# Nikhil-AI-Labs/Image-Super-Resolution

Measured on AMD Instinct MI355X. Metric: SR output megapixels/s (x4, 510x340 LR -> 2040x1360, full 4-expert + 7-phase fusion), higher is better.
Workload: dtype f32 (GEMM/conv products as 3-term split-bf16 MFMA, fp32 accumulate)

## Files before the change

image-super-resolution_amd/csrc/ffsr_attn.hip:

```cpp
#include "ffsr_common.h"

namespace {

struct WinArgs {
  const float* qkv;
  const float* bias;
  float* out;
  int ldq, ldo, C, H, W, ws, shift, heads, hd, hdp, masked;
  float scale;
};

__device__ __forceinline__ int region_id(int p, int n, int ws, int shift) {
  return p < n - ws ? 0 : (p < n - shift ? 1 : 2);
}

template <int DT, int QT>
__global__ __launch_bounds__(256, (QT == 1 ? (DT == 1 ? 4 : (DT == 2 ? 3 : 2)) : (DT <= 2 ? 2 : 1))) void window_attn_kernel(WinArgs p) {
  extern __shared__ __attribute__((aligned(16))) float lds[];
  constexpr int NGMAX = 4 * DT;
  constexpr int WS = 16, N = WS * WS;
  const int QS = p.hdp + 4;
  float* KV = lds;
  int* tok_pix = reinterpret_cast<int*>(KV + 128 * QS + 64);
  int* tok_reg = tok_pix + N;
// ... 525 lines not shown
  for (int d = 0; d < HD; ++d) {
    q[d] = row[d];
    k[d] = row[heads * HD + d];
    Vs[lane][d] = row[2 * heads * HD + d];
  }
  const float kn = inv_norm(k, HD);
#pragma unroll
  for (int d = 0; d < HD; ++d) Ks[lane][d] = k[d] * kn;
  if (lane < NA) {
    const int ay = wy * AW + lane / AW, ax = wx * AW + lane % AW;
    const float* ar = anchor + (((size_t)b * (H / 2) + ay) * (W / 2) + ax) * lda + head * HD;
    float a[HD];
#pragma unroll
    for (int d = 0; d < HD; ++d) a[d] = ar[d];
    const float an = inv_norm(a, HD);
#pragma unroll
    for (int d = 0; d < HD; ++d) As[lane][d] = a[d] * an;
  }
  __syncthreads();
  {
    const int a = lane & 15, kq = lane >> 4;
    const float l1 = logit1[head];
    float s[16];
    float m = -3.0e38f;
#pragma unroll
    for (int jj = 0; jj < 16; ++jj) {
      const int j = kq * 16 + jj;
      float acc = 0.f;
#pragma unroll
      for (int d = 0; d < HD; ++d) acc = fmaf(As[a][d], Ks[j][d], acc);
      acc = acc * l1 + bias1T[((size_t)head * N + j) * NA + a];
      s[jj] = acc;
      m = fmaxf(m, acc);
    }
    m = fmaxf(m, __shfl_xor(m, 16, 64));
    m = fmaxf(m, __shfl_xor(m, 32, 64));
    float sum = 0.f;
#pragma unroll
    for (int jj = 0; jj < 16; ++jj) {
      s[jj] = expf(s[jj] - m);
      sum += s[jj];
    }
    sum += __shfl_xor(sum, 16, 64);
    sum += __shfl_xor(sum, 32, 64);
    const float inv = 1.0f / sum;
#pragma unroll
    for (int jj = 0; jj < 16; ++jj) P1[a][kq * 16 + jj] = s[jj] * inv;
  }
  __syncthreads();
  for (int i = lane; i < NA * HD; i += 64) {
    const int a = i / HD, d = i - a * HD;
    float acc = 0.f;
    for (int j = 0; j < N; ++j) acc = fmaf(P1[a][j], Vs[j][d], acc);
    Gs[a][d] = acc;
  }
  __syncthreads();
  const float qn = inv_norm(q, HD) * logit2[head];
  float s2[NA];
  float m2 = -3.0e38f;
#pragma unroll
  for (int a = 0; a < NA; ++a) {
    float acc = 0.f;
#pragma unroll
    for (int d = 0; d < HD; ++d) acc = fmaf(q[d], As[a][d], acc);
    acc = acc * qn + bias2T[((size_t)head * NA + a) * N + lane];
    s2[a] = acc;
    m2 = fmaxf(m2, acc);
  }
  float sum2 = 0.f;
#pragma unroll
  for (int a = 0; a < NA; ++a) {
    s2[a] = expf(s2[a] - m2);
    sum2 += s2[a];
  }
  const float inv2 = 1.0f / sum2;
  float* orow = out + pix * ldo + ocol0 + head * HD;
#pragma unroll
  for (int d = 0; d < HD; ++d) {
    float acc = 0.f;
#pragma unroll
    for (int a = 0; a < NA; ++a) acc = fmaf(s2[a], Gs[a][d], acc);
    orow[d] = acc * inv2;
  }
}

template <int T>
__global__ __launch_bounds__(256) void pixel_mha_kernel(
    const float* __restrict__ qkv, int ldq, float* __restrict__ out, int ldo, long long S,
                                 int E, int heads, unsigned drop_thr, float keep_scale, unsigned long long seed) {
  constexpr int HD = 16;
  long long idx = (long long)blockIdx.x * blockDim.x + threadIdx.x;
  if (idx >= S * T * heads) return;
  const int h = (int)(idx % heads);
  const long long st = idx / heads;
  const long long seq = st / T;
  const float* qrow = qkv + st * ldq + h * HD;
  float q[HD];
#pragma unroll
  for (int d = 0; d < HD; d += 4) {
    floatx4 v = *reinterpret_cast<const floatx4*>(qrow + d);
    q[d] = v[0] * 0.25f; q[d + 1] = v[1] * 0.25f; q[d + 2] = v[2] * 0.25f; q[d + 3] = v[3] * 0.25f;
  }
  float s[T];
  float m = -3.0e38f;
#pragma unroll
  for (int j = 0; j < T; ++j) {
    const float* krow = qkv + (seq * T + j) * ldq + E + h * HD;
    float acc = 0.f;
#pragma unroll
    for (int d = 0; d < HD; d += 4) {
      floatx4 v = *reinterpret_cast<const floatx4*>(krow + d);
      acc = fmaf(q[d], v[0], acc); acc = fmaf(q[d + 1], v[1], acc);
      acc = fmaf(q[d + 2], v[2], acc); acc = fmaf(q[d + 3], v[3], acc);
    }
    s[j] = acc;
    m = fmaxf(m, acc);
  }
  float sum = 0.f;
#pragma unroll
  for (int j = 0; j < T; ++j) {
    s[j] = expf(s[j] - m);
    sum += s[j];
  }
  const float inv = 1.0f / sum;
  float o[HD];
#pragma unroll
  for (int d = 0; d < HD; ++d) o[d] = 0.f;
#pragma unroll
  for (int j = 0; j < T; ++j) {
    const float* vrow = qkv + (seq * T + j) * ldq + 2 * E + h * HD;
    float pj = s[j] * inv;
    if (drop_thr) {
      const unsigned long long e = (((unsigned long long)seq * heads + h) * T + (unsigned long long)(st - seq * T)) * T + j;
      pj = ffsr_rng_u32(seed, e) >= drop_thr ? pj * keep_scale : 0.f;
    }
#pragma unroll
    for (int d = 0; d < HD; d += 4) {
      floatx4 v = *reinterpret_cast<const floatx4*>(vrow + d);
      o[d] = fmaf(pj, v[0], o[d]); o[d + 1] = fmaf(pj, v[1], o[d + 1]);
      o[d + 2] = fmaf(pj, v[2], o[d + 2]); o[d + 3] = fmaf(pj, v[3], o[d + 3]);
    }
  }
  float* orow = out + st * ldo + h * HD;
#pragma unroll
  for (int d = 0; d < HD; d += 4) {
    floatx4 v = {o[d], o[d + 1], o[d + 2], o[d + 3]};
    *reinterpret_cast<floatx4*>(orow + d) = v;
  }
}

inline bool grid_ok(long long y) { return y > 0 && y <= 65535; }

}

#define ST ((hipStream_t)stream)

extern "C" int ffsr_window_attn_f32(const float* qkv, int ldq, const float* bias, float* out, int ldo, int B, int H, int W,
                                    int C, int heads, int ws, int shift, float scale, int variant, void* stream) {
  FFSR_CHECK(qkv && bias && out && B > 0 && heads > 0 && C % heads == 0);
  FFSR_CHECK(ws > 0 && H % ws == 0 && W % ws == 0 && (ws * ws) % 64 == 0 && ws * ws <= 256);
  FFSR_CHECK(shift >= 0 && shift < ws && ldq >= 3 * C && ldo >= C);
  const int hd = C / heads;
  FFSR_CHECK(hd <= 128);
  WinArgs a;
  a.qkv = qkv; a.bias = bias; a.out = out; a.ldq = ldq; a.ldo = ldo; a.C = C; a.H = H; a.W = W; a.ws = ws;
  a.shift = shift; a.heads = heads; a.hd = hd; a.hdp = (hd + 7) / 8 * 8; a.masked = shift > 0; a.scale = scale;
// ... 2 lines not shown
  FFSR_CHECK(grid_ok((H / ws) * (W / ws) * B));
  if (variant == 0 || variant == 4) {
    const int KS = (hd + 15) / 16, DTx = (KS + 1) / 2;
    const size_t ldsx = (size_t)2 * 64 * (KS * 32 + 16) + (size_t)2 * DTx * 32 * 136 + N * 4 + N +
                        (size_t)(2 * ws - 1) * (2 * ws - 1) * 4;
    const bool wide = variant == 4;
    dim3 gridx((unsigned)(heads * (H / ws) * (W / ws) * B * (wide ? 1 : 2)));
#define LAUNCH_X3(K)                                                                                                  \
  {                                                                                                                   \
    if (ldsx > 64 * 1024) {                                                                                           \
      (void)hipFuncSetAttribute((const void*)window_attn_x3_kernel<K, 4>, hipFuncAttributeMaxDynamicSharedMemorySize, \
                                (int)ldsx);                                                                           \
      (void)hipFuncSetAttribute((const void*)window_attn_x3_kernel<K, 8>, hipFuncAttributeMaxDynamicSharedMemorySize, \
                                (int)ldsx);                                                                           \
    }                                                                                                                 \
    if (wide) FFSR_LAUNCH((window_attn_x3_kernel<K, 8>), gridx, dim3(512), ldsx, ST, a);                        \
    else FFSR_LAUNCH((window_attn_x3_kernel<K, 4>), gridx, dim3(256), ldsx, ST, a);                             \
  }
    switch (KS) {
      case 1: LAUNCH_X3(1); break;
      case 2: LAUNCH_X3(2); break;
      case 3: LAUNCH_X3(3); break;
      case 4: LAUNCH_X3(4); break;
      case 5: LAUNCH_X3(5); break;
      case 6: LAUNCH_X3(6); break;
      case 7: LAUNCH_X3(7); break;
      default: LAUNCH_X3(8); break;
    }
#undef LAUNCH_X3
    return ffsr_launch_status();
  }
  const size_t lds = (size_t)(128 * (a.hdp + 4) + 64) * 4 + 2 * N * 4 + (size_t)(2 * ws - 1) * (2 * ws - 1) * 4;
  FFSR_CHECK(lds <= 160 * 1024);
  const int DT = (hd + 31) / 32;
  const int QT = variant == 2 ? 2 : 1;
  dim3 grid(heads, (H / ws) * (W / ws) * B, QT == 1 ? 2 : 1);
#define LAUNCH_WIN(D, Q)                                                                                            \
  {                                                                                                                 \
    if (lds > 64 * 1024)                                                                                            \
      (void)hipFuncSetAttribute((const void*)window_attn_kernel<D, Q>, hipFuncAttributeMaxDynamicSharedMemorySize, \
                                (int)lds);                                                                          \
    FFSR_LAUNCH((window_attn_kernel<D, Q>), grid, dim3(256), lds, ST, a);                                     \
  }
  switch (DT * 10 + QT) {
    case 11: LAUNCH_WIN(1, 1); break;
    case 12: LAUNCH_WIN(1, 2); break;
    case 21: LAUNCH_WIN(2, 1); break;
    case 22: LAUNCH_WIN(2, 2); break;
    case 31: LAUNCH_WIN(3, 1); break;
    case 32: LAUNCH_WIN(3, 2); break;
    case 41: LAUNCH_WIN(4, 1); break;
    default: LAUNCH_WIN(4, 2); break;
  }
#undef LAUNCH_WIN
  return ffsr_launch_status();
}

extern "C" int ffsr_grl_window_attn_f32(const float* qkv, int ldq, int col0, const float* biasT, const float* logit,
                                        float* out, int ldo, int ocol0, int B, int H, int W, int heads, int hd, int shift,
                                        void* stream) {
  FFSR_CHECK(qkv && biasT && logit && out && B > 0 && H % 8 == 0 && W % 8 == 0 && heads > 0 && shift >= 0 && shift < 8);
  dim3 grid((unsigned)((H / 8) * (W / 8) * B * heads));
  switch (hd) {
    case 30: FFSR_LAUNCH(grl_window_kernel<30>, grid, dim3(64), 0, ST, qkv, ldq, col0, biasT, logit, out, ldo, ocol0, H, W, heads, shift); break;
    case 10: FFSR_LAUNCH(grl_window_kernel<10>, grid, dim3(64), 0, ST, qkv, ldq, col0, biasT, logit, out, ldo, ocol0, H, W, heads, shift); break;
    default: return FFSR_EINVAL;
  }
  return ffsr_launch_status();
}

extern "C" int ffsr_grl_stripe_attn_f32(const float* qkv, int ldq, int col0, const float* anchor, int lda,
                                        const float* bias1T, const float* bias2T, const float* logit1, const float* logit2,
                                        float* out, int ldo, int ocol0, int B, int H, int W, int heads, int hd, void* stream) {
  FFSR_CHECK(qkv && anchor && bias1T && bias2T && logit1 && logit2 && out && B > 0 && H % 8 == 0 && W % 8 == 0 && heads > 0);
  dim3 grid((unsigned)((H / 8) * (W / 8) * B * heads));
  switch (hd) {
    case 30: FFSR_LAUNCH(grl_stripe_kernel<30>, grid, dim3(64), 0, ST, qkv, ldq, col0, anchor, lda, bias1T, bias2T, logit1, logit2, out, ldo, ocol0, H, W, heads); break;
    case 10: FFSR_LAUNCH(grl_stripe_kernel<10>, grid, dim3(64), 0, ST, qkv, ldq, col0, anchor, lda, bias1T, bias2T, logit1, logit2, out, ldo, ocol0, H, W, heads); break;
    default: return FFSR_EINVAL;
  }
  return ffsr_launch_status();
}

extern "C" int ffsr_pixel_mha_f32(const float* qkv, int ldq, float* out, int ldo, long long S, int T, int E, int heads,
                                  float p_drop, long long seed,
                                  void* stream) {
  FFSR_CHECK(qkv && out && S > 0 && heads > 0 && E == heads * 16 && (ldq % 4) == 0 && (ldo % 4) == 0);
  FFSR_CHECK(((uintptr_t)qkv & 15) == 0 && ((uintptr_t)out & 15) == 0);
  FFSR_CHECK(p_drop >= 0.f && p_drop < 1.f);
  const unsigned thr = ffsr_drop_threshold(p_drop);
  const float ks = 1.0f / (1.0f - p_drop);
  long long n = S * T * heads;
  dim3 grid((unsigned)((n + 255) / 256));
  switch (T) {
    case 9: FFSR_LAUNCH(pixel_mha_kernel<9>, grid, dim3(256), 0, ST, qkv, ldq, out, ldo, S, E, heads, thr, ks, (unsigned long long)seed); break;
    case 4: FFSR_LAUNCH(pixel_mha_kernel<4>, grid, dim3(256), 0, ST, qkv, ldq, out, ldo, S, E, heads, thr, ks, (unsigned long long)seed); break;
    default: return FFSR_EINVAL;
  }
  return ffsr_launch_status();
}
```

image-super-resolution_amd/ops.py:

```python
from __future__ import annotations

import math
import os
from dataclasses import dataclass
from typing import Optional

import torch

from . import hip

ACT_NONE, ACT_GELU, ACT_RELU, ACT_LRELU, ACT_SIGMOID, ACT_SILU = range(6)

_ENV_MODE = os.environ.get("FFSR_GEMM_MODE", "bf16x3")
GEMM_MODE = "bf16x3" if _ENV_MODE == "bf16" else _ENV_MODE


WEIGHT_LO = os.environ.get("FFSR_WEIGHT_LO", "1") != "0"


def set_weight_lo(on: bool):
    global WEIGHT_LO
    WEIGHT_LO = bool(on)


# ... 728 lines not shown
    B, H, W, C = x.shape
    n = max(1, min(256, H * W // 64))
    part = torch.empty(B, n, C, device=x.device)
    out = torch.empty(B, C, device=x.device)
    hip.call("ffsr_channel_attention_f32", _ptr(x), ld(x), _ptr(part), n, _ptr(a1.wgt), a1.wgt.shape[1], _ptr(a1.bias),
             _ptr(a3.wgt), a3.wgt.shape[1], _ptr(a3.bias), _ptr(out), B, H * W, C, a1.N, _stream())
    return out


@dataclass
class DwConv:
    w: torch.Tensor
    bias: Optional[torch.Tensor]
    KH: int
    KW: int
    ph: int
    pw: int


def pack_dwconv(w: torch.Tensor, b, device, pad=None) -> DwConv:
    C, one, KH, KW = w.shape
    assert one == 1
    ph, pw = (KH // 2, KW // 2) if pad is None else pad
    return DwConv(w.detach().float().reshape(C, KH * KW).t().contiguous().to(device),
                  None if b is None else b.detach().float().contiguous().to(device), KH, KW, ph, pw)


def dwconv2d(x, dw: DwConv, act=ACT_NONE, out=None):
    B, H, W, C = x.shape
    if out is None:
        out = _like(x)
    hip.call("ffsr_dwconv2d_f32", _ptr(x), ld(x), _ptr(dw.w), _ptr(dw.bias), _ptr(out), ld(out), B, H, W, C, dw.KH,
             dw.KW, dw.ph, dw.pw, act, _stream())
    return out


def dw3x3_gate_pool(x, dw: DwConv):
    B, H, W, C2 = x.shape
    C = C2 // 2
    out = new_map(B, H, W, C, x.device)
    n = _nchunk_gate(H * W)
    part = torch.empty(B, n, C, device=x.device)
    pooled = torch.empty(B, C, device=x.device)
    hip.call("ffsr_dw3x3_gate_pool_f32", _ptr(x), ld(x), _ptr(dw.w), _ptr(dw.bias), _ptr(out), ld(out), _ptr(pooled),
             _ptr(part), B, H, W, C, n, _stream())
    return out, pooled


def bilinear(x, Ho, Wo, mul=1.0, out=None, accumulate=False):
    B, Hi, Wi, C = x.shape
    if out is None:
        out = new_map(B, Ho, Wo, C, x.device)
    hip.call("ffsr_bilinear_f32", _ptr(x), ld(x), _ptr(out), ld(out), B, Hi, Wi, Ho, Wo, C, float(mul),
             int(accumulate), _stream())
    return out


def bicubic_up(x, scale=4, out=None):
    B, H, W, C = x.shape
    if out is None:
        out = new_map(B, H * scale, W * scale, C, x.device)
    hip.call("ffsr_bicubic_up_f32", _ptr(x), ld(x), _ptr(out), ld(out), B, H, W, C, scale, _stream())
    return out


def avgpool2(x, out=None):
    B, H, W, C = x.shape
    if out is None:
        out = new_map(B, H // 2, W // 2, C, x.device)
    hip.call("ffsr_avgpool2_f32", _ptr(x), ld(x), _ptr(out), ld(out), B, H, W, C, _stream())
    return out


def window_attn(qkv, bias, B, H, W, C, heads, ws, shift, scale, out=None, variant=None):
    if out is None:
        out = torch.empty(B * H * W, C, device=qkv.device)
    if variant is None:
        variant = 0 if GEMM_MODE == "bf16x3" else 3
    hip.call("ffsr_window_attn_f32", _ptr(qkv), _mat(qkv)[3], _ptr(bias), _ptr(out), _mat(out)[3], B, H, W, C, heads,
             ws, shift, float(scale), variant, _stream())
    return out


def grl_window_attn(qkv, col0, biasT, logit, out, ocol0, B, H, W, heads, hd, shift):
    hip.call("ffsr_grl_window_attn_f32", _ptr(qkv), _mat(qkv)[3], col0, _ptr(biasT), _ptr(logit), _ptr(out),
             _mat(out)[3], ocol0, B, H, W, heads, hd, shift, _stream())
    return out


def grl_stripe_attn(qkv, col0, anchor, bias1T, bias2T, logit1, logit2, out, ocol0, B, H, W, heads, hd):
    hip.call("ffsr_grl_stripe_attn_f32", _ptr(qkv), _mat(qkv)[3], col0, _ptr(anchor), ld(anchor), _ptr(bias1T),
             _ptr(bias2T), _ptr(logit1), _ptr(logit2), _ptr(out), _mat(out)[3], ocol0, B, H, W, heads, hd, _stream())
    return out


def pixel_mha(qkv, S, T, E, heads, out=None, p_drop=0.0, seed=0):
    if out is None:
        out = torch.empty(S * T, E, device=qkv.device)
    hip.call("ffsr_pixel_mha_f32", _ptr(qkv), _mat(qkv)[3], _ptr(out), _mat(out)[3], S, T, E, heads, float(p_drop), int(seed),
             _stream())
    return out


def scan_chunk(L: int, waves_per_chunk: int = 24) -> int:
    if L >= 64 * 1024:
        best = None
        for c in range(192, 513, 8):
            n = (L + c - 1) // c
            cost = -(-(n * waves_per_chunk) // 4096) * c
            if best is None or cost < best[0]:
                best = (cost, c)
        return best[1]
    c = 32
    while c * 2 <= min(1024, L // 512):
        c *= 2
    return c


SCAN_PAIRS = os.environ.get("FFSR_SCAN_PAIRS", "0") == "1"


def selective_scan4(u, xdbl, dtw, dtb, A, Dv, B, H, W, Dm, R, chunk=None, pairs=None):
    L = H * W
    pairs = (SCAN_PAIRS and L >= 16384) if pairs is None else pairs
    nk = 2 if pairs else 4
    chunk = chunk or scan_chunk(L, nk * B * ((Dm + 63) // 64))
    nchunk = (L + chunk - 1) // chunk
    y = torch.empty(nk, B * L, Dm, device=u.device)
    hstate = torch.empty(B, nk, nchunk, Dm, 16, device=u.device)
    decay = torch.empty_like(hstate)
    hip.call("ffsr_selective_scan4_pairs_f32" if pairs else "ffsr_selective_scan4_f32", _ptr(u), _mat(u)[3], _ptr(xdbl), _mat(xdbl)[3], _ptr(dtw), _ptr(dtb), _ptr(A),
             _ptr(Dv), _ptr(y), Dm, _ptr(hstate), _ptr(decay), B, H, W, Dm, R, 16, chunk, _stream())
    return y


def mamba_norm_gate(y4, z, gamma, beta, eps=1e-5, out=None, out_planes=None, want_f32=True):
    nd, M, C = y4.shape
    assert nd in (2, 4)
    if out_planes is True:
        out_planes = Planes(1, 1, M, C, y4.device)
    if out is None and (want_f32 or out_planes is None):
        out = torch.empty(M, C, device=y4.device)
    hip.call("ffsr_mamba_norm_gate_planes_f32" if nd == 4 else "ffsr_mamba_norm_gate_pairs_f32", _ptr(y4), M * C, C, _ptr(z), _mat(z)[3], _ptr(gamma), _ptr(beta), float(eps),
             _ptr(out), 0 if out is None else _mat(out)[3], None if out_planes is None else _ptr(out_planes.hi),
             None if out_planes is None else _ptr(out_planes.lo), 0 if out_planes is None else out_planes.Cp, M, C, _stream())
    if out_planes is not None:
        return (out, out_planes) if out is not None else out_planes
    return out


def dct_bands(img, D, masks, scale, bands):
    B, H, W, _ = img.shape
    hip.call("ffsr_dct_bands_f32", _ptr(img), ld(img), _ptr(D), _ptr(masks), _ptr(scale), _ptr(bands), 36, B, H, W,
             _stream())


def dwt_db4(img, lo, hi):
    B, H, W, _ = img.shape
    Hd, Wd = (H + 6) // 2 + 1, (W + 6) // 2 + 1
    sub = zeros(B, Hd, Wd, 16, device=img.device)
    hip.call("ffsr_dwt_db4_f32", _ptr(img), ld(img), _ptr(lo), _ptr(hi), _ptr(sub), B, H, W, _stream())
    return sub


def fft_bands(img, twW, twH, mask, scale, bands):
    B, H, W, _ = img.shape
    work = torch.empty(10 * B * 3 * H * (W // 2 + 1), device=img.device)
    hip.call("ffsr_fft_bands_f32", _ptr(img), ld(img), _ptr(twW), _ptr(twH), _ptr(mask), _ptr(scale), _ptr(work),
             _ptr(bands), 36, B, H, W, _stream())


def selector_gates(raw, diff, temperature):
    B, h, w, _ = raw.shape
    gates = torch.empty(B, h, w, 4, device=raw.device)
# ... 92 lines not shown
```

include/ffsr.h:

```cpp
#ifndef FFSR_H
#define FFSR_H

#ifdef __cplusplus
extern "C" {
#endif

#define FFSR_OK 0
#define FFSR_EINVAL (-1)
#define FFSR_ELAUNCH (-2)

int ffsr_conv2d_f32(const float* in, const float* wgt, const float* bias, float* out, const float* res,
                    const float* cvec, const float* rvec, const float* akscale, int B, int H, int W, int Cin, int ldi,
                    int N, int ldo, int ldr, int KH, int KW, int stride, int pad_h, int pad_w, int act, float slope,
                    float cscale, float rscale, int shuffle, int akrows, int tile_hint, void* stream);

int ffsr_set_gemm_terms(int terms);

int ffsr_conv2d_bf16x3(const float* in, const void* wgt_hi, const void* wgt_lo, int ldw, int n_rows_padded,
                       const float* zeros, const float* bias, float* out, const float* res, const float* cvec,
                       const float* rvec, const float* akscale, int B, int H, int W, int Cin, int ldi, int N, int ldo,
                       int ldr, int KH, int KW, int stride, int pad_h, int pad_w, int act, float slope, float cscale,
                       float rscale, int shuffle, int akrows, int bn, void* stream);

int ffsr_conv2d_planes(const void* a_hi, const void* a_lo, int Cp, const void* wgt_hi, const void* wgt_lo,
// ... 7 lines not shown
                       const float* be2, const float* res2, int ldr2, float* out, int ldo, void* out_hi, void* out_lo,
                       int ldp, long long M, int K, int N, int steps, int mode, int pre_ln, float eps1, float eps2,
                       float cscale, float rscale, int waves, void* stream);

int ffsr_tok_chain_tail_f32(const float* x, int ldx, const void* w1, const float* b1, const void* w2, const float* b2,
                            const float* res, int ldr, float* out, int ldo, long long M, int K, int N, int steps, int mode,
                            int pre_ln, float eps1, const void* w3, const float* b3, const float* res3, int ldr3, float* out3,
                            int ldo3, int N3, int act3, float slope3, float cscale3, float rscale3, int waves, void* stream);

int ffsr_tok_head_chain_f32(const float* a, int lda, const float* ascale, const void* w0, const float* b0, const float* g0,
                            const float* be0, float eps0, const float* hres, int ldhr, const float* hres2, int ldhr2,
                            const float* hvec2, int rows_per_batch, const void* w1, const float* b1, const void* w2,
                            const float* b2, const float* g2, const float* be2, float eps2, float* out, int ldo, void* out_hi,
                            void* out_lo, int ldp, long long M, int K, int steps, int mode, int pre_ln, float eps1,
                            const void* w3, const float* b3, const float* res3, int ldr3, float* out3, int ldo3, int N3,
                            int act3, float slope3, float cscale3, float rscale3, int waves, void* stream);

int ffsr_tok_proj_f32(const float* x, long long xstride, int xdirs, int ldx, const float* z, int ldz, const float* pg,
                      const float* pb, float peps, const void* w0, const float* b0, const float* cvec, const float* res,
                      int ldr, const float* rvec, const float* g2, const float* be2, float eps2, float* out, int ldo,
                      int out_pre_ln, void* out_hi, void* out_lo, int ldp, long long M, int K, int N, float cscale,
                      float rscale, int waves, void* stream);

int ffsr_tok_gemm_f32(const float* x, int ldx, const void* w1, const float* b1, const float* cvec, float* out, int ldo,
                      void* out_hi, void* out_lo, int ldp, long long M, int K, int N, int pre_ln, float eps1, int act,
                      float slope, float cscale, int waves, void* stream);

int ffsr_split_planes(const float* x, int ldx, void* hi, void* lo, int ldp, long long M, int C, void* stream);

int ffsr_layernorm_f32(const float* x, int ldx, const float* gamma, const float* beta, float eps, float* out, int ldo,
                       const float* res1, int ldr1, const float* res2, int ldr2, int M, int C, void* stream);

int ffsr_layernorm_planes_f32(const float* x, int ldx, const float* gamma, const float* beta, float eps, float* out,
                              int ldo, void* out_hi, void* out_lo, int ldp, const float* res1, int ldr1,
                              const float* res2, int ldr2, const float* res2_vec, int rows_per_batch, int M, int C,
                              void* stream);

int ffsr_unary_f32(const float* x, int ldx, float* out, int ldo, long long M, int C, int act, float slope, float pre,
                   float alpha, float beta, const float* cscale, const float* cbias, int do_clamp, float lo, float hi,
                   void* stream);

int ffsr_scale_add_f32(const float* a, int lda, const float* avec, const float* b, int ldb, const float* bvec,
                       int rows_per_batch, float* out, int ldo, long long M, int C, float alpha, float beta, void* stream);

int ffsr_mul_add_f32(const float* a, int lda, const float* b, int ldb, int bmode, const float* c, int ldc, float* out,
                     int ldo, long long M, int C, float alpha, float gamma, void* stream);

int ffsr_colmean_f32(const float* x, int ldx, float* out, float* part, int B, int R, int C, int nchunk, void* stream);

int ffsr_channel_attention_f32(const float* x, int ldx, float* part, int nchunk, const float* w1, int ldw1, const float* b1,
                               const float* w2, int ldw2, const float* b2, float* out, int B, int R, int C, int sq, void* stream);

int ffsr_dwconv2d_f32(const float* in, int ldi, const float* w, const float* bias, float* out, int ldo, int B, int H,
                      int W, int C, int KH, int KW, int pad_h, int pad_w, int act, void* stream);

int ffsr_dw3x3_gate_pool_f32(const float* in, int ldi, const float* w, const float* bias, float* out, int ldo,
                             float* pooled, float* part, int B, int H, int W, int C, int nchunk, void* stream);

int ffsr_bilinear_f32(const float* in, int ldi, float* out, int ldo, int B, int Hi, int Wi, int Ho, int Wo, int C,
                      float mul, int accumulate, void* stream);
int ffsr_bicubic_up_f32(const float* in, int ldi, float* out, int ldo, int B, int H, int W, int C, int scale,
                        void* stream);
int ffsr_avgpool2_f32(const float* in, int ldi, float* out, int ldo, int B, int H, int W, int C, void* stream);

int ffsr_u8_to_f32(const unsigned char* in, float* out, int ldo, long long M, int C, void* stream);
int ffsr_f32_to_u8(const float* in, int ldi, unsigned char* out, long long M, int C, void* stream);
int ffsr_pad_reflect_f32(const float* in, int ldi, float* out, int ldo, int B, int H, int W, int Hp, int Wp, int C,
                         void* stream);
int ffsr_crop_f32(const float* in, int ldi, float* out, int ldo, int B, int H, int W, int Ho, int Wo, int C,
                  int do_clamp, void* stream);

int ffsr_dihedral_f32(const float* in, int ldi, float* out, int ldo, int B, int Hi, int Wi, int Ho, int Wo, int C,
                      int ay_i, int ay_j, int cy, int ax_i, int ax_j, int cx, float scale, int accumulate, void* stream);

int ffsr_window_attn_f32(const float* qkv, int ldq, const float* bias, float* out, int ldo, int B, int H, int W, int C,
                         int heads, int ws, int shift, float scale, int variant, void* stream);

int ffsr_grl_window_attn_f32(const float* qkv, int ldq, int col0, const float* biasT, const float* logit, float* out,
                             int ldo, int ocol0, int B, int H, int W, int heads, int hd, int shift, void* stream);

int ffsr_grl_stripe_attn_f32(const float* qkv, int ldq, int col0, const float* anchor, int lda, const float* bias1T,
                             const float* bias2T, const float* logit1, const float* logit2, float* out, int ldo,
                             int ocol0, int B, int H, int W, int heads, int hd, void* stream);

int ffsr_pixel_mha_f32(const float* qkv, int ldq, float* out, int ldo, long long S, int T, int E, int heads, float p_drop,
                       long long seed, void* stream);

int ffsr_selective_scan4_f32(const float* u, int ldu, const float* xdbl, int ldx, const float* dtw, const float* dtb,
                             const float* A, const float* Dv, float* y, int ldy, float* hstate, float* decay, int B,
                             int H, int W, int Dm, int R, int d_state, int chunk, void* stream);
int ffsr_selective_scan4_pairs_f32(const float* u, int ldu, const float* xdbl, int ldx, const float* dtw, const float* dtb,
                                   const float* A, const float* Dv, float* y, int ldy, float* hstate, float* decay, int B,
                                   int H, int W, int Dm, int R, int d_state, int chunk, void* stream);
int ffsr_mamba_norm_gate_f32(const float* y, long long ystride, int ldy, const float* z, int ldz, const float* gamma,
                             const float* beta, float eps, float* out, int ldo, int M, int C, void* stream);
int ffsr_mamba_norm_gate_pairs_f32(const float* y, long long ystride, int ldy, const float* z, int ldz, const float* gamma,
                                   const float* beta, float eps, float* out, int ldo, void* out_hi, void* out_lo, int ldp,
                                   int M, int C, void* stream);

int ffsr_mamba_norm_gate_planes_f32(const float* y, long long ystride, int ldy, const float* z, int ldz,
                                    const float* gamma, const float* beta, float eps, float* out, int ldo, void* out_hi,
                                    void* out_lo, int ldp, int M, int C, void* stream);

int ffsr_dct_bands_f32(const float* img, int ldi, const float* D, const float* masks, const float* scale, float* bands,
                       int ldb, int B, int H, int W, void* stream);
int ffsr_dwt_db4_f32(const float* img, int ldi, const float* lo, const float* hi, float* sub, int B, int H, int W,
                     void* stream);
int ffsr_fft_bands_f32(const float* img, int ldi, const float* twW, const float* twH, const float* mask,
                       const float* scale, float* work, float* bands, int ldb, int B, int H, int W, void* stream);

int ffsr_selector_gates_f32(const float* raw, int ldr, const float* diff, int ldd, const float* temperature,
                            float* gates, int ldg, long long M, void* stream);
int ffsr_modulate_f32(const float* t_lr, int ldt, const float* w2, const float* b2, const float* img, int ldi,
                      float* out, int ldo, int B, int h, int w, int Hh, int Wh, void* stream);
int ffsr_fusion_route_f32(const float* enh, int lde, const float* hier, int ldh, const float* routing, int ldr,
                          const float* fw, const float* gates, int ldg, const float* diff, int ldd, float* out, int ldo,
                          int B, int h, int w, int Hh, int Wh, void* stream);
int ffsr_edge_final_f32(const float* sr, int lds, const float* edge, int lde, const float* gate, int ldg,
                        const float* strength, const float* lr, int ldl, const float* rscale, float* out, int ldo, int B,
                        int h, int w, int Hh, int Wh, void* stream);

int ffsr_conv3x3_thin_f32(const float* in, int ldi, const float* wgt, const float* bias, float* out, int ldo, const float* res,
                          int ldr, int B, int H, int W, int Cin, int N, int act, float slope, float cscale, float rscale,
                          void* stream);

int ffsr_ssim_map_f32(const float* mu1, const float* mu2, const float* e11, const float* e22, const float* e12, int ld,
                      float* out, int ldo, long long M, void* stream);

int ffsr_u8_planes(const unsigned char* img, int H, int W, int crop, int y_channel, unsigned char* planes, void* stream);
int ffsr_psnr_ssim_u8(const unsigned char* pa, const unsigned char* pb, int P, int Hc, int Wc, double* partial,
                      int n_partial, double* out, void* stream);

int ffsr_l1_clamp_loss_f32(const float* sr, int ldsr, const float* hr, int ldhr, float* grad, int ldg, float* partial,
                           int n_partial, float* loss, long long M, int C, float loss_scale, void* stream);
int ffsr_sumsq_f32(const float* x, long long n, float* partial, int n_partial, float* out, void* stream);
int ffsr_adamw_ema_f32(float* param, const float* grad, float* exp_avg, float* exp_avg_sq, float* ema, long long n,
                       const float* grad_sumsq, float max_norm, float lr, float beta1, float beta2, float eps,
                       float weight_decay, int step, float ema_decay, void* stream);


int ffsr_zero_f32(float* p, long long n, void* stream);

int ffsr_pack_conv_f32(const float* w, int N, int Cin, int KH, int KW, int transpose, float* dst_f32, int Cp, void* dst_hi,
                       void* dst_lo, int rows_pad, int ldw, void* stream);
int ffsr_pack_dwconv_f32(const float* w, int C, int KH, int KW, int flip, float* dst, void* stream);

int ffsr_conv_wgrad_f32(const float* x, int ldx, const float* dy, int ldy, float* dw, float* dbias, float* partial,
                        long long partial_floats, int B, int H, int W, int Cin, int N, int KH, int KW, int pad_h, int pad_w,
                        void* stream);
int ffsr_conv_wgrad_bf16x3(const float* x, int ldx, const float* dy, int ldy, float* dw, float* dbias, float* partial,
                           long long partial_floats, int B, int H, int W, int Cin, int N, int KH, int KW, int pad_h, int pad_w,
                           void* stream);
int ffsr_conv_wgrad_bf16x3_planes(const void* x_hi, const void* x_lo, int ldp, const float* dy, int ldy, const void* dy_hi,
                                  const void* dy_lo, int ldq, float* dw, float* dbias, float* partial, long long partial_floats,
                                  int B, int H, int W, int Cin, int N, int KH, int KW, int pad_h, int pad_w, void* stream);
int ffsr_dwconv_wgrad_f32(const float* x, int ldx, const float* dy, int ldy, float* dw, float* partial, int nchunk, int B, int H,
                          int W, int C, int KH, int KW, int pad_h, int pad_w, void* stream);

int ffsr_act_bwd_f32(const float* dy, int ldy, const float* ref, int ldr, float* dx, int ldx, long long M, int C, int act,
                     float slope, int from_output, float alpha, int accumulate, void* stream);
int ffsr_act_bwd_planes_f32(const float* dy, int ldy, const float* ref, int ldr, void* out_hi, void* out_lo, int ldp, long long M,
                            int C, int act, float slope, int from_output, float alpha, void* stream);
int ffsr_axpby_dev_f32(const float* a, int lda, const float* sa, float alpha, const float* b, int ldb, const float* sb,
                       float beta, float* out, int ldo, long long M, int C, void* stream);
int ffsr_dot_acc_f32(const float* a, int lda, const float* b, int ldb, long long M, int C, double* partial, int n_partial,
                     float* out, float scale, int accumulate, void* stream);
// ... 43 lines not shown
```

Before: 9.271.

## Add MFMA-based GRL window and stripe attention kernels staged through LDS

Adds new GRL window and stripe attention kernels that compute QK^T and PV with fp32 16x16x4 MFMA instructions. Each block handles one 8x8 window for all heads, staging qkv rows and anchors in LDS with coalesced paired loads and precomputing inverse norms. This replaces the per-head scalar-FMA kernels, which used a 64-thread block per window-head. The new path is on by default in bf16x3 mode and costs large dynamic LDS per block, which may limit occupancy.

```diff
diff --git a/image-super-resolution_amd/csrc/ffsr_attn.hip b/image-super-resolution_amd/csrc/ffsr_attn.hip
--- a/image-super-resolution_amd/csrc/ffsr_attn.hip
+++ b/image-super-resolution_amd/csrc/ffsr_attn.hip
@@ -631,6 +631,322 @@
     for (int a = 0; a < NA; ++a) acc = fmaf(s2[a], Gs[a][d], acc);
     orow[d] = acc * inv2;
   }
+}
+
+__device__ __forceinline__ int grl_rs(int rw) { return rw + ((4 - rw) % 8 + 8) % 8; }
+
+template <bool PAIR, int CP>
+__device__ __forceinline__ void grl_stage_rows(const float* __restrict__ qkv, int ldq, int col0, int RW, int RS,
+                                               const int* pix, float* X, int lane, int wave) {
+  const int PR = RW >> 1;
+  float2 r[16][CP];
+#pragma unroll
+  for (int j = 0; j < 16; ++j) {
+    const float* src = qkv + (size_t)pix[wave + 4 * j] * ldq + col0;
+#pragma unroll
+    for (int c = 0; c < CP; ++c) {
+      const int cc = min(lane + 64 * c, PR - 1);
+      if (PAIR) r[j][c] = *reinterpret_cast<const float2*>(src + 2 * cc);
+      else r[j][c] = float2{src[2 * cc], src[2 * cc + 1]};
+    }
+  }
+#pragma unroll
+  for (int j = 0; j < 16; ++j)
+#pragma unroll
+    for (int c = 0; c < CP; ++c)
+      if (lane + 64 * c < PR) *reinterpret_cast<float2*>(X + (wave + 4 * j) * RS + 2 * (lane + 64 * c)) = r[j][c];
+}
+
+__device__ __forceinline__ void grl_store_rows(float* __restrict__ out, int ldo, int ocol0, int CB, int RS, const int* pix,
+                                               const float* X, int lane, int wave) {
+  const bool pair = ((ldo | ocol0) & 1) == 0 && (reinterpret_cast<uintptr_t>(out) & 7) == 0;
+  if (pair) {
+#pragma unroll 4
+    for (int j = 0; j < 16; ++j) {
+      const int t = wave + 4 * j;
+      float* dst = out + (size_t)pix[t] * ldo + ocol0;
+      for (int c = lane; c < (CB >> 1); c += 64) *reinterpret_cast<float2*>(dst + 2 * c) = *reinterpret_cast<const float2*>(X + t * RS + 2 * c);
+    }
+  } else {
+#pragma unroll 4
+    for (int j = 0; j < 16; ++j) {
+      const int t = wave + 4 * j;
+      float* dst = out + (size_t)pix[t] * ldo + ocol0;
+      for (int c = lane; c < CB; c += 64) dst[c] = X[t * RS + c];
+    }
+  }
+}
+
+template <int HD>
+__device__ __forceinline__ float grl_inv_norm_lds(const float* v) {
+  float s = 0.f;
+#pragma unroll
+  for (int d = 0; d < HD; ++d) s = fmaf(v[d], v[d], s);
+  return 1.0f / fmaxf(sqrtf(s), 1e-12f);
+}
+
+template <int HD>
+__device__ __forceinline__ floatx4 grl_st_tile(const float* Kc, int RS, int t, const float (&qv)[(HD + 3) / 4], int l15, int g) {
+  floatx4 acc = {0.f, 0.f, 0.f, 0.f};
+  const float* kr = Kc + (16 * t + l15) * RS;
+#pragma unroll
+  for (int s = 0; s < (HD + 3) / 4; ++s) {
+    const int d = 4 * s + g;
+    const float a = d < HD ? kr[min(d, HD - 1)] : 0.f;
+    acc = __builtin_amdgcn_mfma_f32_16x16x4f32(a, qv[s], acc, 0, 0, 0);
+  }
+  return acc;
+}
+
+__device__ __forceinline__ float grl_softmax64(floatx4 (&s)[4]) {
+  float m = -3.0e38f;
+#pragma unroll
+  for (int t = 0; t < 4; ++t)
+#pragma unroll
+    for (int i = 0; i < 4; ++i) m = fmaxf(m, s[t][i]);
+  m = fmaxf(m, __shfl_xor(m, 16, 64));
+  m = fmaxf(m, __shfl_xor(m, 32, 64));
+  float sum = 0.f;
+#pragma unroll
+  for (int t = 0; t < 4; ++t)
+#pragma unroll
+    for (int i = 0; i < 4; ++i) {
+      s[t][i] = expf(s[t][i] - m);
+      sum += s[t][i];
+    }
+  sum += __shfl_xor(sum, 16, 64);
+  sum += __shfl_xor(sum, 32, 64);
+  return 1.0f / sum;
+}
+
+template <int HD>
+__device__ __forceinline__ void grl_pv(const float* Vc, int RS, const floatx4 (&p)[4], floatx4 (&o)[(HD + 15) / 16], int l15,
+                                       int g) {
+#pragma unroll
+  for (int dt = 0; dt < (HD + 15) / 16; ++dt) {
+    o[dt] = floatx4{0.f, 0.f, 0.f, 0.f};
+    const float* vc = Vc + min(16 * dt + l15, HD - 1);
+#pragma unroll
+    for (int t = 0; t < 4; ++t)
+#pragma unroll
+      for (int i = 0; i < 4; ++i) o[dt] = __builtin_amdgcn_mfma_f32_16x16x4f32(vc[(16 * t + 4 * g + i) * RS], p[t][i], o[dt], 0, 0, 0);
+  }
+}
+
+template <int HD>
+__device__ __forceinline__ void grl_put_ot(float* X, int RS, int row, int col, const floatx4 (&o)[(HD + 15) / 16], float scale,
+                                           int g) {
+#pragma unroll
+  for (int dt = 0; dt < (HD + 15) / 16; ++dt)
+#pragma unroll
+    for (int i = 0; i < 4; ++i) {
+      const int d = 16 * dt + 4 * g + i;
+      if (d < HD) X[row * RS + col + d] = o[dt][i] * scale;
+    }
+}
+
+template <int HD, bool PAIR, int CP>
+__global__ __launch_bounds__(256) void grl_window_mfma_kernel(const float* __restrict__ qkv, int ldq, int col0,
+                                                              const float* __restrict__ biasT, const float* __restrict__ logit,
+                                                              float* __restrict__ out, int ldo, int ocol0, int H, int W,
+                                                              int heads, int shift) {
+  constexpr int WS = 8, N = 64, KS = (HD + 3) / 4, DT = (HD + 15) / 16;
+  extern __shared__ __attribute__((aligned(16))) float lds[];
+  const int CB = heads * HD, RW = 3 * CB, RS = grl_rs(RW);
+  float* X = lds;
+  float* nrm = X + N * RS;
+  int* pix = reinterpret_cast<int*>(nrm + 2 * heads * N);
+  int* reg = pix + N;
+  const int tid = threadIdx.x, lane = tid & 63, wave = tid >> 6, l15 = lane & 15, g = lane >> 4;
+  const int nwx = W / WS, nwy = H / WS;
+  const int win = blockIdx.x % (nwx * nwy), b = blockIdx.x / (nwx * nwy);
+  const int wy = win / nwx, wx = win % nwx;
+  if (tid < N) {
+    const int ys = wy * WS + tid / WS, xs = wx * WS + tid % WS;
+    int y = ys + shift, x = xs + shift;
+    if (y >= H) y -= H;
+    if (x >= W) x -= W;
+    pix[tid] = (b * H + y) * W + x;
+    reg[tid] = shift ? region_id(ys, H, WS, shift) * 3 + region_id(xs, W, WS, shift) : 0;
+  }
+  __syncthreads();
+  const int q = 16 * wave + l15;
+  float bv[16];
+  auto load_bias = [&](int h) {
+    const float* bt = biasT + (size_t)h * N * N + (4 * g) * N + q;
+#pragma unroll
+    for (int j = 0; j < 16; ++j) bv[j] = bt[((j >> 2) * 16 + (j & 3)) * N];
+  };
+  load_bias(0);
+  grl_stage_rows<PAIR, CP>(qkv, ldq, col0, RW, RS, pix, X, lane, wave);
+  __syncthreads();
+  for (int i = tid; i < 2 * heads * N; i += 256) {
+    const int t = i % N, ph = i / N;
+    nrm[i] = grl_inv_norm_lds<HD>(X + t * RS + ph * HD);
+  }
+  __syncthreads();
+  const int myreg = reg[q];
+  const bool use_mask = shift && (wy == nwy - 1 || wx == nwx - 1);
+#pragma unroll 1
+  for (int h = 0; h < heads; ++h) {
+    float qv[KS];
+#pragma unroll
+    for (int s = 0; s < KS; ++s) {
+      const int d = 4 * s + g;
+      qv[s] = d < HD ? X[q * RS + h * HD + min(d, HD - 1)] : 0.f;
+    }
+    float bh[16];
+#pragma unroll
+    for (int j = 0; j < 16; ++j) bh[j] = bv[j];
+    load_bias(min(h + 1, heads - 1));
+    const float* rk = nrm + (heads + h) * N;
+    const float qs = nrm[h * N + q] * logit[h];
+    floatx4 s[4];
+#pragma unroll
+    for (int t = 0; t < 4; ++t) {
+      s[t] = grl_st_tile<HD>(X + CB + h * HD, RS, t, qv, l15, g);
+      const floatx4 kn = *reinterpret_cast<const floatx4*>(rk + 16 * t + 4 * g);
+#pragma unroll
+      for (int i = 0; i < 4; ++i) {
+        const int key = 16 * t + 4 * g + i;
+        float v = s[t][i] * qs * kn[i] + bh[4 * t + i];
+        if (use_mask && reg[key] != myreg) v += -100.0f;
+        s[t][i] = v;
+      }
+    }
+    const float inv = grl_softmax64(s);
+    floatx4 o[DT];
+    grl_pv<HD>(X + 2 * CB + h * HD, RS, s, o, l15, g);
+    grl_put_ot<HD>(X, RS, q, h * HD, o, inv, g);
+  }
+  __syncthreads();
+  grl_store_rows(out, ldo, ocol0, CB, RS, pix, X, lane, wave);
+}
+
+template <int HD, bool PAIR, int CP>
+__global__ __launch_bounds__(256) void grl_stripe_mfma_kernel(const float* __restrict__ qkv, int ldq, int col0,
+                                                              const float* __restrict__ anchor, int lda,
+                                                              const float* __restrict__ bias1T, const float* __restrict__ bias2T,
+                                                              const float* __restrict__ logit1, const float* __restrict__ logit2,
+                                                              float* __restrict__ out, int ldo, int ocol0, int H, int W, int heads) {
+  constexpr int WS = 8, N = 64, AW = 4, NA = 16, KS = (HD + 3) / 4, DT = (HD + 15) / 16;
+  extern __shared__ __attribute__((aligned(16))) float lds[];
+  const int CB = heads * HD, RW = 3 * CB, RS = grl_rs(RW), AS = grl_rs(CB);
+  float* X = lds;
+  float* A = X + N * RS;
+  float* nrm = A + NA * AS;
+  int* pix = reinterpret_cast<int*>(nrm + 2 * heads * N + heads * NA);
+  const int tid = threadIdx.x, lane = tid & 63, wave = tid >> 6, l15 = lane & 15, g = lane >> 4;
+  const int nwx = W / WS, nwy = H / WS;
+  const int win = blockIdx.x % (nwx * nwy), b = blockIdx.x / (nwx * nwy);
+  const int wy = win / nwx, wx = win % nwx;
+  if (tid < N) pix[tid] = (b * H + wy * WS + tid / WS) * W + wx * WS + tid % WS;
+  __syncthreads();
+  float ar[8];
+#pragma unroll
+  for (int j = 0; j < 8; ++j) {
+    const int i = min(tid + 256 * j, NA * CB - 1), a = i / CB, c = i - a * CB;
+    ar[j] = anchor[(((size_t)b * (H / 2) + wy * AW + a / AW) * (W / 2) + wx * AW + a % AW) * lda + c];
+  }
+  float b1v[16], b2v[4];
+  auto load_bias1 = [&](int h) {
+    const float* bt = bias1T + (size_t)h * N * NA + (4 * g) * NA + l15;
+#pragma unroll
+    for (int j = 0; j < 16; ++j) b1v[j] = bt[((j >> 2) * 16 + (j & 3)) * NA];
+  };
+  const int q = 16 * wave + l15;
+  auto load_bias2 = [&](int h) {
+#pragma unroll
+    for (int i = 0; i < 4; ++i) b2v[i] = bias2T[((size_t)h * NA + 4 * g + i) * N + q];
+  };
+  load_bias1(min(wave, heads - 1));
+  load_bias2(0);
+  grl_stage_rows<PAIR, CP>(qkv, ldq, col0, RW, RS, pix, X, lane, wave);
+#pragma unroll
+  for (int j = 0; j < 8; ++j) {
+    const int i = tid + 256 * j;
+    if (i < NA * CB) A[(i / CB) * AS + i % CB] = ar[j];
+  }
+  __syncthreads();
+  for (int i = tid; i < 2 * heads * N + heads * NA; i += 256) {
+    if (i < 2 * heads * N) nrm[i] = grl_inv_norm_lds<HD>(X + (i % N) * RS + (i / N) * HD);
+    else {
+      const int j = i - 2 * heads * N;
+      nrm[i] = grl_inv_norm_lds<HD>(A + (j % NA) * AS + (j / NA) * HD);
+    }
+  }
+  __syncthreads();
+  const float* ra = nrm + 2 * heads * N;
+#pragma unroll 1
+  for (int h = wave; h < heads; h += 4) {
+    float av[KS];
+#pragma unroll
+    for (int s = 0; s < KS; ++s) {
+      const int d = 4 * s + g;
+      av[s] = d < HD ? A[l15 * AS + h * HD + min(d, HD - 1)] : 0.f;
+    }
+    if (h != wave) load_bias1(h);
+    const float* rk = nrm + (heads + h) * N;
+    const float as = ra[h * NA + l15] * logit1[h];
+    floatx4 s[4];
+#pragma unroll
+    for (int t = 0; t < 4; ++t) {
+      s[t] = grl_st_tile<HD>(X + CB + h * HD, RS, t, av, l15, g);
+      const floatx4 kn = *reinterpret_cast<const floatx4*>(rk + 16 * t + 4 * g);
+#pragma unroll
+      for (int i = 0; i < 4; ++i) s[t][i] = s[t][i] * as * kn[i] + b1v[4 * t + i];
+    }
+    const float inv = grl_softmax64(s);
+    floatx4 o[DT];
+    grl_pv<HD>(X + 2 * CB + h * HD, RS, s, o, l15, g);
+    grl_put_ot<HD>(X, RS, l15, CB + h * HD, o, inv, g);
+  }
+  __syncthreads();
+#pragma unroll 1
+  for (int h = 0; h < heads; ++h) {
+    float bh[4];
+#pragma unroll
+    for (int i = 0; i < 4; ++i) bh[i] = b2v[i];
+    load_bias2(min(h + 1, heads - 1));
+    floatx4 s = {0.f, 0.f, 0.f, 0.f};
+#pragma unroll
+    for (int st = 0; st < KS; ++st) {
+      const int d = 4 * st + g, dc = min(d, HD - 1);
+      const float a = d < HD ? A[l15 * AS + h * HD + dc] : 0.f;
+      const float qv = d < HD ? X[q * RS + h * HD + dc] : 0.f;
+      s = __builtin_amdgcn_mfma_f32_16x16x4f32(a, qv, s, 0, 0, 0);
+    }
+    const float qs = nrm[h * N + q] * logit2[h];
+    const floatx4 an = *reinterpret_cast<const floatx4*>(ra + h * NA + 4 * g);
+    float m = -3.0e38f;
+#pragma unroll
+    for (int i = 0; i < 4; ++i) {
+      s[i] = s[i] * an[i] * qs + bh[i];
+      m = fmaxf(m, s[i]);
+    }
+    m = fmaxf(m, __shfl_xor(m, 16, 64));
+    m = fmaxf(m, __shfl_xor(m, 32, 64));
+    float sum = 0.f;
+#pragma unroll
+    for (int i = 0; i < 4; ++i) {
+      s[i] = expf(s[i] - m);
+      sum += s[i];
+    }
+    sum += __shfl_xor(sum, 16, 64);
+    sum += __shfl_xor(sum, 32, 64);
+    floatx4 o[DT];
+    const float* gc = X + CB + h * HD;
+#pragma unroll
+    for (int dt = 0; dt < DT; ++dt) {
+      o[dt] = floatx4{0.f, 0.f, 0.f, 0.f};
+      const float* gcd = gc + min(16 * dt + l15, HD - 1);
+#pragma unroll
+      for (int i = 0; i < 4; ++i) o[dt] = __builtin_amdgcn_mfma_f32_16x16x4f32(gcd[(4 * g + i) * RS], s[i], o[dt], 0, 0, 0);
+    }
+    grl_put_ot<HD>(X, RS, q, h * HD, o, 1.0f / sum, g);
+  }
+  __syncthreads();
+  grl_store_rows(out, ldo, ocol0, CB, RS, pix, X, lane, wave);
 }
 
 template <int T>
@@ -799,6 +1115,83 @@
   return ffsr_launch_status();
 }
 
+namespace {
+int grl_mfma_cp(int heads, int hd) {
+  if (hd != 10 && hd != 30) return 0;
+  const int pr = 3 * heads * hd / 2;
+  return pr <= 64 ? 1 : (pr <= 128 ? 2 : (pr <= 192 ? 3 : 0));
+}
+
+template <int HD, bool PAIR, int CP>
+int grl_window_mfma_launch(size_t lds, hipStream_t stream, const float* qkv, int ldq, int col0, const float* biasT,
+                           const float* logit, float* out, int ldo, int ocol0, int B, int H, int W, int heads, int shift) {
+  static unsigned long long attr_set = 0;
+  const void* fn = (const void*)grl_window_mfma_kernel<HD, PAIR, CP>;
+  if (ffsr_allow_dynamic_lds(&fn, 1, 160 * 1024, &attr_set) != FFSR_OK) return FFSR_ELAUNCH;
+  FFSR_LAUNCH((grl_window_mfma_kernel<HD, PAIR, CP>), dim3((unsigned)((H / 8) * (W / 8) * B)), dim3(256), lds, stream, qkv, ldq,
+              col0, biasT, logit, out, ldo, ocol0, H, W, heads, shift);
+  return ffsr_launch_status();
+}
+
+template <int HD, bool PAIR, int CP>
+int grl_stripe_mfma_launch(size_t lds, hipStream_t stream, const float* qkv, int ldq, int col0, const float* anchor, int lda,
+                           const float* bias1T, const float* bias2T, const float* logit1, const float* logit2, float* out,
+                           int ldo, int ocol0, int B, int H, int W, int heads) {
+  static unsigned long long attr_set = 0;
+  const void* fn = (const void*)grl_stripe_mfma_kernel<HD, PAIR, CP>;
+  if (ffsr_allow_dynamic_lds(&fn, 1, 160 * 1024, &attr_set) != FFSR_OK) return FFSR_ELAUNCH;
+  FFSR_LAUNCH((grl_stripe_mfma_kernel<HD, PAIR, CP>), dim3((unsigned)((H / 8) * (W / 8) * B)), dim3(256), lds, stream, qkv, ldq,
+              col0, anchor, lda, bias1T, bias2T, logit1, logit2, out, ldo, ocol0, H, W, heads);
+  return ffsr_launch_status();
+}
+}
+
+#define GRL_MFMA_DISPATCH(LAUNCH, ...)                                                               \
+  switch ((hd == 30 ? 100 : 0) + (pair ? 10 : 0) + cp) {                                            \
+    case 111: return LAUNCH<30, true, 1>(__VA_ARGS__);                                               \
+    case 112: return LAUNCH<30, true, 2>(__VA_ARGS__);                                               \
+    case 113: return LAUNCH<30, true, 3>(__VA_ARGS__);                                               \
+    case 101: return LAUNCH<30, false, 1>(__VA_ARGS__);                                              \
+    case 102: return LAUNCH<30, false, 2>(__VA_ARGS__);                                              \
+    case 103: return LAUNCH<30, false, 3>(__VA_ARGS__);                                              \
+    case 11: return LAUNCH<10, true, 1>(__VA_ARGS__);                                                \
+    case 12: return LAUNCH<10, true, 2>(__VA_ARGS__);                                                \
+    case 13: return LAUNCH<10, true, 3>(__VA_ARGS__);                                                \
+    case 1: return LAUNCH<10, false, 1>(__VA_ARGS__);                                                \
+    case 2: return LAUNCH<10, false, 2>(__VA_ARGS__);                                                \
+    default: return LAUNCH<10, false, 3>(__VA_ARGS__);                                               \
+  }
+
+extern "C" int ffsr_grl_window_attn_mfma_f32(const float* qkv, int ldq, int col0, const float* biasT, const float* logit,
+                                             float* out, int ldo, int ocol0, int B, int H, int W, int heads, int hd, int shift,
+                                             void* stream) {
+  FFSR_CHECK(qkv && biasT && logit && out && B > 0 && H % 8 == 0 && W % 8 == 0 && heads > 0 && shift >= 0 && shift < 8);
+  const int cp = grl_mfma_cp(heads, hd);
+  FFSR_CHECK(cp > 0 && col0 >= 0 && ldq >= col0 + 3 * heads * hd && ocol0 >= 0 && ldo >= ocol0 + heads * hd);
+  const bool pair = ((ldq | col0) & 1) == 0 && (reinterpret_cast<uintptr_t>(qkv) & 7) == 0;
+  const int rs = 3 * heads * hd + ((4 - 3 * heads * hd) % 8 + 8) % 8;
+  const size_t lds = ((size_t)64 * rs + 2 * heads * 64) * 4 + 2 * 64 * 4;
+  FFSR_CHECK(lds <= 160 * 1024);
+  GRL_MFMA_DISPATCH(grl_window_mfma_launch, lds, ST, qkv, ldq, col0, biasT, logit, out, ldo, ocol0, B, H, W, heads, shift)
+}
+
+extern "C" int ffsr_grl_stripe_attn_mfma_f32(const float* qkv, int ldq, int col0, const float* anchor, int lda,
+                                             const float* bias1T, const float* bias2T, const float* logit1,
+                                             const float* logit2, float* out, int ldo, int ocol0, int B, int H, int W,
+                                             int heads, int hd, void* stream) {
+  FFSR_CHECK(qkv && anchor && bias1T && bias2T && logit1 && logit2 && out && B > 0 && H % 8 == 0 && W % 8 == 0 && heads > 0);
+  const int cp = grl_mfma_cp(heads, hd);
+  FFSR_CHECK(cp > 0 && col0 >= 0 && ldq >= col0 + 3 * heads * hd && ocol0 >= 0 && ldo >= ocol0 + heads * hd &&
+             lda >= heads * hd);
+  const bool pair = ((ldq | col0) & 1) == 0 && (reinterpret_cast<uintptr_t>(qkv) & 7) == 0;
+  const int cb = heads * hd, rs = 3 * cb + ((4 - 3 * cb) % 8 + 8) % 8, as = cb + ((4 - cb) % 8 + 8) % 8;
+  const size_t lds = ((size_t)64 * rs + 16 * as + 2 * heads * 64 + heads * 16) * 4 + 64 * 4;
+  FFSR_CHECK(lds <= 160 * 1024);
+  GRL_MFMA_DISPATCH(grl_stripe_mfma_launch, lds, ST, qkv, ldq, col0, anchor, lda, bias1T, bias2T, logit1, logit2, out, ldo,
+                    ocol0, B, H, W, heads)
+}
+#undef GRL_MFMA_DISPATCH
+
 extern "C" int ffsr_pixel_mha_f32(const float* qkv, int ldq, float* out, int ldo, long long S, int T, int E, int heads,
                                   float p_drop, long long seed,
                                   void* stream) {
diff --git a/image-super-resolution_amd/ops.py b/image-super-resolution_amd/ops.py
--- a/image-super-resolution_amd/ops.py
+++ b/image-super-resolution_amd/ops.py
@@ -834,14 +834,24 @@
     return out
 
 
-def grl_window_attn(qkv, col0, biasT, logit, out, ocol0, B, H, W, heads, hd, shift):
-    hip.call("ffsr_grl_window_attn_f32", _ptr(qkv), _mat(qkv)[3], col0, _ptr(biasT), _ptr(logit), _ptr(out),
+GRL_ATTN_MFMA = os.environ.get("FFSR_GRL_ATTN_MFMA", "1") != "0"
+
+
+def _grl_mfma(mfma: Optional[bool]) -> bool:
+    return (GRL_ATTN_MFMA and GEMM_MODE == "bf16x3") if mfma is None else bool(mfma)
+
+
+def grl_window_attn(qkv, col0, biasT, logit, out, ocol0, B, H, W, heads, hd, shift, mfma: Optional[bool] = None):
+    fn = "ffsr_grl_window_attn_mfma_f32" if _grl_mfma(mfma) else "ffsr_grl_window_attn_f32"
+    hip.call(fn, _ptr(qkv), _mat(qkv)[3], col0, _ptr(biasT), _ptr(logit), _ptr(out),
              _mat(out)[3], ocol0, B, H, W, heads, hd, shift, _stream())
     return out
 
 
-def grl_stripe_attn(qkv, col0, anchor, bias1T, bias2T, logit1, logit2, out, ocol0, B, H, W, heads, hd):
-    hip.call("ffsr_grl_stripe_attn_f32", _ptr(qkv), _mat(qkv)[3], col0, _ptr(anchor), ld(anchor), _ptr(bias1T),
+def grl_stripe_attn(qkv, col0, anchor, bias1T, bias2T, logit1, logit2, out, ocol0, B, H, W, heads, hd,
+                    mfma: Optional[bool] = None):
+    fn = "ffsr_grl_stripe_attn_mfma_f32" if _grl_mfma(mfma) else "ffsr_grl_stripe_attn_f32"
+    hip.call(fn, _ptr(qkv), _mat(qkv)[3], col0, _ptr(anchor), ld(anchor), _ptr(bias1T),
              _ptr(bias2T), _ptr(logit1), _ptr(logit2), _ptr(out), _mat(out)[3], ocol0, B, H, W, heads, hd, _stream())
     return out
 
diff --git a/include/ffsr.h b/include/ffsr.h
--- a/include/ffsr.h
+++ b/include/ffsr.h
@@ -113,6 +113,12 @@
 int ffsr_grl_stripe_attn_f32(const float* qkv, int ldq, int col0, const float* anchor, int lda, const float* bias1T,
                              const float* bias2T, const float* logit1, const float* logit2, float* out, int ldo,
                              int ocol0, int B, int H, int W, int heads, int hd, void* stream);
+
+int ffsr_grl_window_attn_mfma_f32(const float* qkv, int ldq, int col0, const float* biasT, const float* logit, float* out,
+                                  int ldo, int ocol0, int B, int H, int W, int heads, int hd, int shift, void* stream);
+int ffsr_grl_stripe_attn_mfma_f32(const float* qkv, int ldq, int col0, const float* anchor, int lda, const float* bias1T,
+                                  const float* bias2T, const float* logit1, const float* logit2, float* out, int ldo,
+                                  int ocol0, int B, int H, int W, int heads, int hd, void* stream);
 
 int ffsr_pixel_mha_f32(const float* qkv, int ldq, float* out, int ldo, long long S, int T, int E, int heads, float p_drop,
                        long long seed, void* stream);
```

Result: no change. 9.339 (median of 6 runs) (+0.7%).
